# muellerlab/agri-fly

Measured on AMD Instinct MI355X. Metric: vehicle-steps/sec @dt=1ms, higher is better.
Workload: dtype f32; 1 GPU; BASELINE config 4 per GPU: 1048576 hovering CF_MINIQUAD vehicles, per-vehicle wind gusts (sigma 0..0.5 N, 100 ms epochs), IMU synthesis + noise at the 500 Hz logic gate, one afe_step call per 1 ms step, state through memory every step; vehicles_per_gpu=1048576, vehicles_total=1048576, steps_per_call=1, stepping=persistent, noise=AFE_SEED_DECORRELATED: the reference's per-vehicle libstdc++ streams, bit-exact, parallelism=contiguous shards, 1 rank(s), no data-path collective

## Files before the change

agri-fly_amd/csrc/afe_kernels.hip:

```cpp
#include <hip/hip_runtime.h>
#include <stdint.h>

#include "afe_device.h"

namespace afe {

__device__ __forceinline__ float fm(float a, float b, float c) { return __builtin_fmaf(a, b, c); }
__device__ __forceinline__ double fm(double a, double b, double c) { return __builtin_fma(a, b, c); }
__device__ __forceinline__ float m_abs(float x) { return fabsf(x); }
__device__ __forceinline__ double m_abs(double x) { return fabs(x); }
__device__ __forceinline__ float m_med3(float x, float lo, float hi) { return __builtin_amdgcn_fmed3f(x, lo, hi); }
__device__ __forceinline__ double m_med3(double x, double lo, double hi) { return x > hi ? hi : (x < lo ? lo : x); }


template <typename R>
__device__ __forceinline__ void rot_matrix(R v0, R v1, R v2, R v3, R M[9]) {
#pragma clang fp contract(off)
  const R r0 = v0 * v0, r1 = v1 * v1, r2 = v2 * v2, r3 = v3 * v3;
  const R a = 2 * v0, b = 2 * v1, c = 2 * v2;
  M[0] = r0 + r1 - r2 - r3;
  M[1] = fm(b, v2, -(a * v3));
  M[2] = fm(b, v3, a * v2);
  M[3] = fm(b, v2, a * v3);
  M[4] = r0 - r1 + r2 - r3;
  M[5] = fm(c, v3, -(a * v1));
  M[6] = fm(b, v3, -(a * v2));
  M[7] = fm(c, v3, a * v1);
  M[8] = r0 - r1 - r2 + r3;
}

template <typename R, typename M>
__device__ __forceinline__ void mat_vec(const M *A, R x, R y, R z, R &ox, R &oy, R &oz) {
#pragma clang fp contract(off)
  ox = fm(R(A[2]), z, fm(R(A[1]), y, R(A[0]) * x));
  oy = fm(R(A[5]), z, fm(R(A[4]), y, R(A[3]) * x));
  oz = fm(R(A[8]), z, fm(R(A[7]), y, R(A[6]) * x));
}

#ifndef AFE_ACCEPT_LOOP
#define AFE_ACCEPT_LOOP 2
#endif

__device__ __forceinline__ uint32_t minstd_next(uint32_t &s) {
  const uint64_t p = (uint64_t)s * 16807u;
  uint32_t r = (uint32_t)(p & 0x7fffffffu) + (uint32_t)(p >> 31);
  if (r >= 2147483647u) r -= 2147483647u;
  s = r;
  return r;
}

__device__ __forceinline__ uint32_t minstd_mul(uint32_t x, uint32_t k) {
  const uint64_t p = (uint64_t)x * k;
  uint32_t r = (uint32_t)(p & 0x7fffffffu) + (uint32_t)(p >> 31);
  if (r >= 2147483647u) r -= 2147483647u;
  return r;
}

__device__ __forceinline__ double canonical53(uint32_t &s) {
#pragma clang fp contract(off)
  double sum = (double)(minstd_next(s) - 1u);
  sum = sum + (double)(minstd_next(s) - 1u) * 2147483646.0;
  const double b = 4611686009837453312.0;
  const double y = 1.0 / 4611686009837453312.0;
  const double q0 = sum * y;
  const double r = __builtin_fma(-q0, b, sum);
  double ret = __builtin_fma(r, y, q0);
  if (ret >= 1.0) ret = 0x1.fffffffffffffp-1;
  return ret;
}

__device__ __forceinline__ double polar_multiplier(double r2) {
#pragma clang fp contract(off)
  double m = __builtin_amdgcn_frexp_mant(r2);
  int e = __builtin_amdgcn_frexp_exp(r2);
  if (m < 0.70710678118654752) { m = m + m; e -= 1; }
  const double f = m - 1.0;
  const double b = 2.0 + f;
  double y = __builtin_amdgcn_rcp(b);
  y = __builtin_fma(y, __builtin_fma(-b, y, 1.0), y);
  y = __builtin_fma(y, __builtin_fma(-b, y, 1.0), y);
  double sq = f * y;
  sq = __builtin_fma(__builtin_fma(-b, sq, f), y, sq);
  const double z = sq * sq;
  double p = 1.0 / 21.0;
  p = __builtin_fma(p, z, 1.0 / 19.0);
  p = __builtin_fma(p, z, 1.0 / 17.0);
  p = __builtin_fma(p, z, 1.0 / 15.0);
  p = __builtin_fma(p, z, 1.0 / 13.0);
  p = __builtin_fma(p, z, 1.0 / 11.0);
  p = __builtin_fma(p, z, 1.0 / 9.0);
  p = __builtin_fma(p, z, 1.0 / 7.0);
  p = __builtin_fma(p, z, 1.0 / 5.0);
  p = __builtin_fma(p, z, 1.0 / 3.0);
  const double two_s = sq + sq;
  const double lnm = __builtin_fma(two_s * z, p, two_s);
  const double ed = (double)e;
  const double ln_r2 = __builtin_fma(ed, 6.93147180369123816490e-01, __builtin_fma(ed, 1.90821492927058770002e-10, lnm));
  const double L = -2.0 * ln_r2;
  const double w = L * r2;
  if (!(w > 0.0)) return 0.0;
  double g = __builtin_amdgcn_rsq(w);
  g = __builtin_fma(g, 0.5 * __builtin_fma(-(w * g), g, 1.0), g);
  g = __builtin_fma(g, 0.5 * __builtin_fma(-(w * g), g, 1.0), g);
  return L * g;
}

__device__ __forceinline__ float polar_multiplier_f32(double r2) {
#pragma clang fp contract(off)
  double m = __builtin_amdgcn_frexp_mant(r2);
  int e = __builtin_amdgcn_frexp_exp(r2);
  if (m < 0.70710678118654752) { m = m + m; e -= 1; }
  const float f = (float)(m - 1.0);
  const float sq = f * __builtin_amdgcn_rcpf(2.0f + f);
  const float z = sq * sq;
  float p = 1.0f / 9.0f;
  p = __builtin_fmaf(p, z, 1.0f / 7.0f);
  p = __builtin_fmaf(p, z, 1.0f / 5.0f);
  p = __builtin_fmaf(p, z, 1.0f / 3.0f);
  const float two_s = sq + sq;
  const float lnm = __builtin_fmaf(two_s * z, p, two_s);
  const float ln_r2 = __builtin_fmaf((float)e, 0.693147182f, lnm);
  const float L = -2.0f * ln_r2;
  if (!(L > 0.0f)) return 0.0f;
  return __builtin_amdgcn_sqrtf(L * __builtin_amdgcn_rcpf((float)r2));
}

__device__ __forceinline__ void polar_candidate(uint32_t &s, double &x, double &y, double &r2) {
#pragma clang fp contract(off)
  x = 2.0 * canonical53(s) - 1.0;
  y = 2.0 * canonical53(s) - 1.0;
  r2 = x * x + y * y;
}

__device__ __forceinline__ void three_accepted(uint32_t &s, uint32_t &st0, uint32_t &st1, uint32_t &st2) {
#pragma clang fp contract(off)
#if AFE_ACCEPT_LOOP == 2
  st0 = s; st1 = s; st2 = s;
  int got = 0;
  const uint32_t kLo = __builtin_bit_cast(uint32_t, 1e-5f), kUp = __builtin_bit_cast(uint32_t, 1.0f - 1e-5f),
                 kTop = __builtin_bit_cast(uint32_t, 1.0f + 1e-5f);
  for (;;) {
    const uint32_t before = s;
    const uint32_t hx = minstd_mul(before, 282475249u);
    const uint32_t hy = minstd_mul(before, 984943658u);
    s = hy;
    const float kInvR = 1.0f / 2147483646.0f;
    const float xf = __builtin_fmaf((float)(hx - 1u), 2.0f * kInvR, -1.0f);
    const float yf = __builtin_fmaf((float)(hy - 1u), 2.0f * kInvR, -1.0f);
    const uint32_t rb = __builtin_bit_cast(uint32_t, __builtin_fmaf(xf, xf, yf * yf));
    bool accept = (rb - (kLo + 1u)) < (kUp - kLo - 1u);
    const bool unsure = !accept && rb <= kTop;
    if (__ballot(unsure)) {
      if (unsure) {
        uint32_t t = before;
        asm volatile("" : "+v"(t));
        double x, y, r2;
        polar_candidate(t, x, y, r2);
        accept = !(r2 > 1.0 || r2 == 0.0);
      }
    }
    if (accept) {
      asm volatile("v_mov_b32 %0, %1\n\tv_mov_b32 %1, %2\n\tv_mov_b32 %2, %3" : "+&v"(st0), "+&v"(st1), "+&v"(st2) : "v"(before));
      got++;
    }
    if (got >= 3) break;
  }
#else
  st0 = s; st1 = s; st2 = s;
  int got = 0;
  while (got < 3) {
    const uint32_t before = s;
    const uint32_t hx = minstd_mul(before, 282475249u);
    const uint32_t hy = minstd_mul(before, 984943658u);
    s = hy;
    const float kInvR = 1.0f / 2147483646.0f;
    const float xf = __builtin_fmaf((float)(hx - 1u), 2.0f * kInvR, -1.0f);
    const float yf = __builtin_fmaf((float)(hy - 1u), 2.0f * kInvR, -1.0f);
    const float r2f = __builtin_fmaf(xf, xf, yf * yf);
    bool accept = r2f < 1.0f - 1e-5f && r2f > 1e-5f;
    const bool unsure = !accept && !(r2f > 1.0f + 1e-5f);
    if (__ballot(unsure)) {
      if (unsure) {
        uint32_t t = before;
        asm volatile("" : "+v"(t));
        double x, y, r2;
        polar_candidate(t, x, y, r2);
        accept = !(r2 > 1.0 || r2 == 0.0);
      }
    }
    const int slot = accept ? got : 3;
    st0 = slot == 0 ? before : st0;
    st1 = slot == 1 ? before : st1;
    st2 = slot == 2 ? before : st2;
    got += accept ? 1 : 0;
  }
#endif
}

__device__ __forceinline__ void six_normals(uint32_t &s, double d[6]) {
#pragma clang fp contract(off)
  uint32_t st0, st1, st2;
  three_accepted(s, st0, st1, st2);
  double x0, y0, r0, x1, y1, r1, x2, y2, r2;
  polar_candidate(st0, x0, y0, r0);
  polar_candidate(st1, x1, y1, r1);
  polar_candidate(st2, x2, y2, r2);
  const double m0 = polar_multiplier(r0);
  const double m1 = polar_multiplier(r1);
  const double m2 = polar_multiplier(r2);
  d[0] = y0 * m0; d[1] = x0 * m0;
  d[2] = y1 * m1; d[3] = x1 * m1;
  d[4] = y2 * m2; d[5] = x2 * m2;
}

__device__ __forceinline__ void six_normals(uint32_t &s, float d[6]) {
#pragma clang fp contract(off)
  uint32_t st0, st1, st2;
  three_accepted(s, st0, st1, st2);
  double x0, y0, r0, x1, y1, r1, x2, y2, r2;
  polar_candidate(st0, x0, y0, r0);
  polar_candidate(st1, x1, y1, r1);
  polar_candidate(st2, x2, y2, r2);
  const float m0 = polar_multiplier_f32(r0);
  const float m1 = polar_multiplier_f32(r1);
  const float m2 = polar_multiplier_f32(r2);
  d[0] = (float)y0 * m0; d[1] = (float)x0 * m0;
  d[2] = (float)y1 * m1; d[3] = (float)x1 * m1;
  d[4] = (float)y2 * m2; d[5] = (float)x2 * m2;
}

__device__ __forceinline__ void philox4x32_10(uint32_t c[4], uint32_t k0, uint32_t k1) {
  const uint32_t M0 = 0xD2511F53u, M1 = 0xCD9E8D57u, W0 = 0x9E3779B9u, W1 = 0xBB67AE85u;
  asm volatile("" : "+s"(k0), "+s"(k1));
#pragma unroll
  for (int r = 0; r < 10; r++) {
    const uint32_t h0 = __umulhi(M0, c[0]), l0 = M0 * c[0], h1 = __umulhi(M1, c[2]), l1 = M1 * c[2];
    c[0] = h1 ^ c[1] ^ k0; c[1] = l1; c[2] = h0 ^ c[3] ^ k1; c[3] = l0;
    k0 += W0; k1 += W1;
  }
}
#define AFE_STREAM_IMU 1u
#define AFE_STREAM_GUST 2u
__device__ __forceinline__ void counter_block(uint64_t seed, uint64_t index, uint32_t stream, uint32_t block, uint64_t ordinal, uint32_t w[4]) {
  w[0] = (uint32_t)index;
  w[1] = (uint32_t)((index >> 32) & 0xffffu) | (stream << 16) | (block << 24);
  w[2] = (uint32_t)ordinal;
  w[3] = (uint32_t)(ordinal >> 32);
  philox4x32_10(w, (uint32_t)seed, (uint32_t)(seed >> 32));
}
__device__ __forceinline__ void box_muller(uint32_t xe, uint32_t xo, float &za, float &zb) {
#pragma clang fp contract(off)
  const float u_r = ((float)(xe >> 9) + 0.5f) * (1.0f / 8388608.0f);
  const float u_a = (float)(xo >> 8) * (1.0f / 16777216.0f);
  float m = __builtin_amdgcn_frexp_mantf(u_r);
  int e = __builtin_amdgcn_frexp_expf(u_r);
  if (m < 0.70710678f) { m = m + m; e -= 1; }
  const float f = m - 1.0f;
  const float sq = f * __builtin_amdgcn_rcpf(2.0f + f);
  const float z = sq * sq;
  float p = 1.0f / 9.0f;
  p = __builtin_fmaf(p, z, 1.0f / 7.0f);
  p = __builtin_fmaf(p, z, 1.0f / 5.0f);
  p = __builtin_fmaf(p, z, 1.0f / 3.0f);
  const float two_s = sq + sq;
  const float lnm = __builtin_fmaf(two_s * z, p, two_s);
  const float ln_u = __builtin_fmaf((float)e, 0.693147182f, lnm);
  const float r = __builtin_amdgcn_sqrtf(-2.0f * ln_u);
  za = r * __builtin_amdgcn_cosf(u_a);
  zb = r * __builtin_amdgcn_sinf(u_a);
}
__device__ __forceinline__ void box_muller(uint32_t xe, uint32_t xo, double &za, double &zb) {
#pragma clang fp contract(off)
  const double u_r = ((double)(xe >> 9) + 0.5) * (1.0 / 8388608.0);
  const double u_a = (double)(xo >> 8) * (1.0 / 16777216.0);
  const double r = sqrt(-2.0 * log(u_r));
  double sn, cs;
  sincos(6.283185307179586476925286766559 * u_a, &sn, &cs);
  za = r * cs;
  zb = r * sn;
}
template <typename N>
__device__ __forceinline__ void counter_six_normals(uint64_t seed, uint64_t index, uint64_t tick, N d[6]) {
  uint32_t a[4], b[4];
  counter_block(seed, index, AFE_STREAM_IMU, 0, tick, a);
  counter_block(seed, index, AFE_STREAM_IMU, 1, tick, b);
  N unused0, unused1;
  box_muller(a[0], a[1], d[0], d[1]);
  box_muller(a[2], a[3], d[2], d[3]);
  box_muller(b[0], b[1], d[4], d[5]);
  (void)unused0; (void)unused1;
}
template <typename R>
__device__ __forceinline__ void gust_force(uint64_t seed, uint64_t index, uint64_t n_global, uint64_t epoch, double sigma_max, R f[3]) {
#pragma clang fp contract(off)
  uint32_t w[4];
  counter_block(seed, index, AFE_STREAM_GUST, 0, epoch, w);
  R z0, z1, z2, z3;
  box_muller(w[0], w[1], z0, z1);
  box_muller(w[2], w[3], z2, z3);
  const R sigma = (R)(sigma_max * (double)index / (double)(n_global > 1 ? n_global - 1 : 1));
  f[0] = sigma * z0; f[1] = sigma * z1; f[2] = sigma * z2;
}

__device__ __forceinline__ void rotvec_to_quat(double rx, double ry, double rz,
                                               double &d0, double &d1, double &d2, double &d3) {
#pragma clang fp contract(off)
  const double theta = sqrt(rx * rx + ry * ry + rz * rz);
  d0 = 1; d1 = 0; d2 = 0; d3 = 0;
  if (!(theta < 4.84813681e-6)) {
    double sn, cs;
    sincos(theta * 0.5, &sn, &cs);
    d0 = cs;
    d1 = sn * (rx / theta);
    d2 = sn * (ry / theta);
    d3 = sn * (rz / theta);
  }
}
__device__ __forceinline__ void rotvec_to_quat(float rx, float ry, float rz,
// ... 289 lines not shown

    R Lx, Ly, Lzz;
    mat_vec<R>(P.I, wx, wy, wz, Lx, Ly, Lzz);
    if (lagged) Lzz = (((Lzz + Lm[0]) + Lm[1]) + Lm[2]) + Lm[3];
    const R cx = fm(wy, Lzz, -(wz * Ly));
    const R cy = fm(wz, Lx, -(wx * Lzz));
    const R cz = fm(wx, Ly, -(wy * Lx));
    R aax, aay, aaz;
    mat_vec<R>(P.Iinv, Tx - cx, Ty - cy, Tz - cz, aax, aay, aaz);

    const R vbx = fm(Rm[6], vz, fm(Rm[3], vy, Rm[0] * vx));
    const R vby = fm(Rm[7], vz, fm(Rm[4], vy, Rm[1] * vx));
    const R vbz = fm(Rm[8], vz, fm(Rm[5], vy, Rm[2] * vx));
    const R Fbx = P.drag[0] * (-vbx);
    const R Fby = P.drag[1] * (-vby);
    const R Fbz = fm(P.drag[2], -vbz, Fz);

    R accx = div_mass(fm(Rm[2], Fbz, fm(Rm[1], Fby, Rm[0] * Fbx)) + fex, P.mass, P.inv_mass);
    R accy = div_mass(fm(Rm[5], Fbz, fm(Rm[4], Fby, Rm[3] * Fbx)) + fey, P.mass, P.inv_mass);
    R accz, nvz;
    if (sizeof(R) == 4) {
      const R rest = fm(Rm[8], P.drag[2] * (-vbz), fm(Rm[7], Fby, Rm[6] * Fbx)) + fez;
      const double accz_d = __builtin_fma((double)Rm[8], P.kf_over_mass_d * W2_d, -9.81) + (double)(rest * P.inv_mass);
      accz = (R)accz_d;
      nvz = (R)((double)vz + (double)dt * accz_d);
    } else {
      accz = R(-9.81) + div_mass(fm(Rm[8], Fbz, fm(Rm[7], Fby, Rm[6] * Fbx)) + fez, P.mass, P.inv_mass);
      nvz = fm(dt, accz, vz);
    }

    const R hdt = R(0.5) * dt;
    R npx = fm(dt, fm(hdt, accx, vx), px);
    R npy = fm(dt, fm(hdt, accy, vy), py);
    R npz = fm(dt, fm(hdt, accz, vz), pz);
    R nvx = fm(dt, accx, vx), nvy = fm(dt, accy, vy);
    R d0, d1, d2, d3;
    rotvec_to_quat(dt * wx, dt * wy, dt * wz, d0, d1, d2, d3);
    R n0 = fm(-d3, q3, fm(-d2, q2, fm(-d1, q1, d0 * q0)));
    R n1 = fm(-d2, q3, fm(d3, q2, fm(d0, q1, d1 * q0)));
    R n2 = fm(d1, q3, fm(d0, q2, fm(-d3, q1, d2 * q0)));
    R n3 = fm(d0, q3, fm(-d1, q2, fm(d2, q1, d3 * q0)));
    R nwx = fm(dt, aax, wx), nwy = fm(dt, aay, wy), nwz = fm(dt, aaz, wz);

    if (RENORM) {
      const R inv = quat_inv_norm(fm(n3, n3, fm(n2, n2, fm(n1, n1, n0 * n0))));
      n0 *= inv; n1 *= inv; n2 *= inv; n3 *= inv;
    }

    if ((npz <= 0) && (nvz < 0)) {
      npz = 0; nvz = 0; accz = 0;
      nwx = 0; nwy = 0; nwz = 0;
    }
    px = npx; py = npy; pz = npz;
    vx = nvx; vy = nvy; vz = nvz;
    q0 = n0; q1 = n1; q2 = n2; q3 = n3;
    wx = nwx; wy = nwy; wz = nwz;

    if (LOGIC && SINGLE && AFE_LOGIC_LOADS_LATE) {
      AFE_ST(R, pos, 0, off, px); AFE_ST(R, pos, 1, off, py); AFE_ST(R, pos, 2, off, pz);
      AFE_ST(R, vel, 0, off, vx); AFE_ST(R, vel, 1, off, vy); AFE_ST(R, vel, 2, off, vz);
      AFE_ST(R, att, 0, off, q0); AFE_ST(R, att, 1, off, q1); AFE_ST(R, att, 2, off, q2); AFE_ST(R, att, 3, off, q3);
      AFE_ST(R, ang_vel, 0, off, wx); AFE_ST(R, ang_vel, 1, off, wy); AFE_ST(R, ang_vel, 2, off, wz);
    }
    if (tick) {
      if (LOGIC && SINGLE && AFE_LOGIC_LOADS_LATE) {
        __builtin_amdgcn_sched_barrier(0);
        AFE_LOAD_LOGIC_STATE();
      }
      float tx_, ty_, tz_;
      mat_vec<float>(P.Rimu, (float)wx, (float)wy, (float)wz, tx_, ty_, tz_);
      gx = tx_ + ng[0]; gy = ty_ + ng[1]; gz = tz_ + ng[2];
      R Rn[9];
      rot_matrix<R>(q0, q1, q2, q3, Rn);
      const R sx = accx + R(0), sy = accy + R(0), sz = accz + R(9.81);
      const R bx = fm(Rn[6], sz, fm(Rn[3], sy, Rn[0] * sx));
      const R by = fm(Rn[7], sz, fm(Rn[4], sy, Rn[1] * sx));
      const R bz = fm(Rn[8], sz, fm(Rn[5], sy, Rn[2] * sx));
      mat_vec<float>(P.Rimu, (float)bx, (float)by, (float)bz, tx_, ty_, tz_);
      ax_m = tx_ + na[0]; ay_m = ty_ + na[1]; az_m = tz_ + na[2];
      have_imu = true;
      if (LOGIC) {
        rates_logic_tick(G, lg, gx, gy, gz, cmd_new);
#pragma unroll
        for (int m = 0; m < 4; m++) { cmd[m] = (R)cmd_new[m]; if (cmd[m] < 0) cmd[m] = 0; }
      }
    }
    if (EACH && step + 1 < n_steps) {
      AFE_ST(R, pos, 0, off, px); AFE_ST(R, pos, 1, off, py); AFE_ST(R, pos, 2, off, pz);
      AFE_ST(R, vel, 0, off, vx); AFE_ST(R, vel, 1, off, vy); AFE_ST(R, vel, 2, off, vz);
      AFE_ST(R, att, 0, off, q0); AFE_ST(R, att, 1, off, q1); AFE_ST(R, att, 2, off, q2); AFE_ST(R, att, 3, off, q3);
      AFE_ST(R, ang_vel, 0, off, wx); AFE_ST(R, ang_vel, 1, off, wy); AFE_ST(R, ang_vel, 2, off, wz);
      if (v.motor_write) { AFE_ST(R, motor, 0, off, ms[0]); AFE_ST(R, motor, 1, off, ms[1]); AFE_ST(R, motor, 2, off, ms[2]); AFE_ST(R, motor, 3, off, ms[3]); }
      if (tick) {
        AFE_ST(float, gyro, 0, off4, gx); AFE_ST(float, gyro, 1, off4, gy); AFE_ST(float, gyro, 2, off4, gz);
        AFE_ST(float, acc, 0, off4, ax_m); AFE_ST(float, acc, 1, off4, ay_m); AFE_ST(float, acc, 2, off4, az_m);
        if (LOGIC) {
#pragma unroll
          for (int m = 0; m < 4; m++) AFE_ST(float, cmd_out, m, off4, cmd_new[m]);
        }
      }
    }
  }

  if (!(LOGIC && SINGLE && AFE_LOGIC_LOADS_LATE)) {
    AFE_ST(R, pos, 0, off, px); AFE_ST(R, pos, 1, off, py); AFE_ST(R, pos, 2, off, pz);
    AFE_ST(R, vel, 0, off, vx); AFE_ST(R, vel, 1, off, vy); AFE_ST(R, vel, 2, off, vz);
    AFE_ST(R, att, 0, off, q0); AFE_ST(R, att, 1, off, q1); AFE_ST(R, att, 2, off, q2); AFE_ST(R, att, 3, off, q3);
    AFE_ST(R, ang_vel, 0, off, wx); AFE_ST(R, ang_vel, 1, off, wy); AFE_ST(R, ang_vel, 2, off, wz);
  }
  if (v.motor_write) {
    AFE_ST(R, motor, 0, off, ms[0]); AFE_ST(R, motor, 1, off, ms[1]); AFE_ST(R, motor, 2, off, ms[2]); AFE_ST(R, motor, 3, off, ms[3]);
  }
  if (have_imu) {
    AFE_ST(float, gyro, 0, off4, gx); AFE_ST(float, gyro, 1, off4, gy); AFE_ST(float, gyro, 2, off4, gz);
    AFE_ST(float, acc, 0, off4, ax_m); AFE_ST(float, acc, 1, off4, ay_m); AFE_ST(float, acc, 2, off4, az_m);
    if (NOISE == 1) AFE_ST(uint32_t, rng, 0, off4, rng);
    if (LOGIC) {
#pragma unroll
      for (int k = 0; k < 3; k++) {
        AFE_STL(float, lpf, k, off4, lg.xm0[k]);
        AFE_STL(float, lpf, 3 + k, off4, lg.xm1[k]);
        AFE_STL(float, lpf, 6 + k, off4, lg.ym0[k]);
        AFE_STL(float, lpf, 9 + k, off4, lg.ym1[k]);
      }
      v.imu_init[(uint32_t)i] = lg.imu_init;
#pragma unroll
      for (int m = 0; m < 4; m++) AFE_ST(float, cmd_out, m, off4, cmd_new[m]);
    }
  }
#undef AFE_LD
#undef AFE_ST
#undef AFE_LDL
#undef AFE_LOAD_LOGIC_STATE
#undef AFE_STL
}

#ifndef AFE_LB_WAVES
#define AFE_LB_WAVES 1
#endif
#ifndef AFE_BLOCK
#define AFE_BLOCK 64
#endif

template <typename R, bool FEXT, bool TEXT, int NOISE, bool LOGIC, bool SINGLE, bool BUF, int CP = 0>
__global__ void __launch_bounds__(AFE_BLOCK, AFE_LB_WAVES)
afe_step_kernel(const StepView<R> v, const DevParams<R> P, const DevLogic G) {
  const unsigned b = CP == 3 ? (blockIdx.x & 7u) * (gridDim.x >> 3) + (blockIdx.x >> 3) : blockIdx.x;
  const int64_t i = v.first + (int64_t)b * AFE_BLOCK + threadIdx.x;
  if (i >= v.end) return;
  run_vehicle<R, FEXT, TEXT, NOISE, LOGIC, SINGLE, BUF, false, (CP > 2 ? 2 : CP)>(v, P, G, i, v.tick_mask, v.n_steps, v.tick_base);
}

template <typename R, bool FEXT, bool TEXT, int NOISE, bool LOGIC, bool BUF>
__global__ void __launch_bounds__(256)
afe_step_kernel_table(const StepView<R> v) {
  extern __shared__ __align__(16) unsigned char lds_raw[];
  const int words_p = v.n_types * (int)(sizeof(DevParams<R>) / 4);
  const int words_g = LOGIC ? v.n_types * (int)(sizeof(DevLogic) / 4) : 0;
  {
    const uint32_t *src = reinterpret_cast<const uint32_t *>(v.table);
    uint32_t *dst = reinterpret_cast<uint32_t *>(lds_raw);
    for (int k = threadIdx.x; k < words_p; k += 256) dst[k] = src[k];
    if (LOGIC) {
      const uint32_t *srcg = reinterpret_cast<const uint32_t *>(v.logic_table);
      for (int k = threadIdx.x; k < words_g; k += 256) dst[words_p + k] = srcg[k];
    }
  }
  __syncthreads();
  const int64_t i = v.first + (int64_t)blockIdx.x * 256 + threadIdx.x;
  if (i >= v.end) return;
  const unsigned t = v.type[(uint32_t)i];
  const DevParams<R> &P = reinterpret_cast<const DevParams<R> *>(lds_raw)[t];
  const DevLogic &G = reinterpret_cast<const DevLogic *>(lds_raw + (size_t)words_p * 4)[LOGIC ? t : 0];
  run_vehicle<R, FEXT, TEXT, NOISE, LOGIC, false, BUF>(v, P, G, i, v.tick_mask, v.n_steps, v.tick_base);
}

template <typename R, bool FEXT, bool TEXT, int NOISE, bool LOGIC, bool BUF>
__global__ void __launch_bounds__(AFE_BLOCK, AFE_LB_WAVES)
afe_step_kernel_wave_types(const StepView<R> v) {
  const int64_t i = v.first + (int64_t)blockIdx.x * AFE_BLOCK + threadIdx.x;
  if (i >= v.end) return;
  const unsigned t = (unsigned)__builtin_amdgcn_readfirstlane((int)v.type[i]);
  const DevParams<R> P = v.table[t];
  DevLogic G = {};
  if (LOGIC) G = v.logic_table[t];
  run_vehicle<R, FEXT, TEXT, NOISE, LOGIC, false, BUF>(v, P, G, i, v.tick_mask, v.n_steps, v.tick_base);
}

typedef unsigned long long u64_t;
__device__ __forceinline__ u64_t ld_agent(const u64_t *p) { return __hip_atomic_load(p, __ATOMIC_RELAXED, __HIP_MEMORY_SCOPE_AGENT); }
__device__ __forceinline__ void st_agent(u64_t *p, u64_t x) { __hip_atomic_store(p, x, __ATOMIC_RELAXED, __HIP_MEMORY_SCOPE_AGENT); }
__device__ __forceinline__ u64_t ld_system(const u64_t *p) { return __hip_atomic_load(p, __ATOMIC_RELAXED, __HIP_MEMORY_SCOPE_SYSTEM); }
__device__ __forceinline__ void st_system(u64_t *p, u64_t x) { __hip_atomic_store(p, x, __ATOMIC_RELAXED, __HIP_MEMORY_SCOPE_SYSTEM); }
typedef unsigned int afe_u32x16 __attribute__((ext_vector_type(16)));
__device__ __forceinline__ u64_t afe_uniform64(unsigned long long a) {
  return ((u64_t)(unsigned)__builtin_amdgcn_readfirstlane((int)(a >> 32)) << 32) | (unsigned)__builtin_amdgcn_readfirstlane((int)a);
}
__device__ __forceinline__ void sld_system_8_1(const u64_t *p0, const u64_t *p1, u64_t (&x)[8], u64_t &y) {
  afe_u32x16 v;
  const u64_t u0 = afe_uniform64((unsigned long long)p0), u1 = afe_uniform64((unsigned long long)p1);
  asm volatile("s_load_dwordx16 %0, %2, 0x0 glc\n\ts_load_dwordx2 %1, %3, 0x0 glc\n\ts_waitcnt lgkmcnt(0)" : "=&s"(v), "=&s"(y) : "s"(u0), "s"(u1) : "memory");
#pragma unroll
  for (int i = 0; i < 8; i++) x[i] = ((u64_t)v[2 * i + 1] << 32) | v[2 * i];
}
__device__ __forceinline__ void sld_system2(const u64_t *p0, const u64_t *p1, u64_t &x0, u64_t &x1) {
  const u64_t u0 = afe_uniform64((unsigned long long)p0), u1 = afe_uniform64((unsigned long long)p1);
  asm volatile("s_load_dwordx2 %0, %2, 0x0 glc\n\ts_load_dwordx2 %1, %3, 0x0 glc\n\ts_waitcnt lgkmcnt(0)" : "=&s"(x0), "=&s"(x1) : "s"(u0), "s"(u1) : "memory");
}
__device__ __forceinline__ u64_t ticks100() { return __builtin_amdgcn_s_memrealtime(); }
__device__ __forceinline__ int ones_from_bit0(u64_t m) { return m == ~0ull ? 64 : (int)__builtin_ctzll(~m); }
__device__ __forceinline__ u64_t entry_index(u64_t e) { return (e >> 2) & ((1ull << 46) - 1); }
__device__ __forceinline__ u64_t entry_stamp(u64_t e, unsigned epoch) { return (e & ((1ull << 48) - 1)) | ((u64_t)(epoch & 0xffffu) << 48); }

__device__ __forceinline__ u64_t *persist_sync_counters(const PersistArgs &a) { return a.done + ((a.n_workers + 15) & ~15) + 16; }

__device__ __forceinline__ void persist_pump(const PersistArgs &a) {
  const int lane = (int)threadIdx.x;
  u64_t p = a.start;
  const u64_t t_start = ticks100();
  u64_t t_fed = t_start;
  u64_t t_moving = t_start;
  u64_t m_seen = a.start;
  u64_t park_pos;
  u64_t err = 0;
  u64_t m = a.start;
  u64_t *const help = a.dev_ring - 1;
  if (lane == 0) st_agent(help, 0);
  for (int w = lane; w < a.n_workers; w += 64) st_agent(a.done + w, a.start);
  st_agent(persist_sync_counters(a) + 16 * lane, 0);
  if (lane == 0) st_agent(persist_sync_counters(a) + 16 * AFE_PERSIST_SYNC_SHARDS, 0);
  __builtin_amdgcn_fence(__ATOMIC_RELEASE, "agent");
  u64_t req_marked = 0;
  u64_t acc = ~0ull;
  int sw = 0;
  u64_t d[8];
  u64_t help_in = 0, help_seen = 0;
  int slice_age = -1;
#pragma unroll
  for (int j = 0; j < 8; j++) d[j] = ~0ull;
  for (;;) {
    const u64_t idx = p + (u64_t)lane;
    u64_t e8[8], req;
    const u64_t slot = p & a.host_mask;
    if (slot + 8 <= a.host_mask + 1) sld_system_8_1(a.host_ring + slot, a.host_status + AFE_PERSIST_SYNCREQ_WORD, e8, req);
    else {
      sld_system2(a.host_ring + slot, a.host_status + AFE_PERSIST_SYNCREQ_WORD, e8[0], req);
#pragma unroll
      for (int i = 1; i < 8; i++) e8[i] = 0;
    }
    const bool news = entry_index(e8[0]) == p + 1;
    bool all8 = true;
#pragma unroll
    for (int i = 0; i < 8; i++) all8 = all8 && entry_index(e8[i]) == p + 1 + (u64_t)i;
    const bool fetch = all8 && p + 64 < m + (u64_t)a.dev_mask + 1;
    u64_t h = 0;
    if (fetch) h = ld_system(a.host_ring + (idx & a.host_mask));
    else {
#pragma unroll
      for (int i = 0; i < 8; i++) h = lane == i ? e8[i] : h;
    }
    const bool tight = p + 192 >= m + (u64_t)a.dev_mask + 1;
    if (slice_age >= (tight ? 0 : 2)) {
#pragma unroll
      for (int j = 0; j < 8; j++) acc = d[j] < acc ? d[j] : acc;
      help_seen = help_in;
      slice_age = -1;
      sw += 512;
      if (sw >= a.n_workers) {
        u64_t r = acc;
#pragma unroll
        for (int o = 32; o > 0; o >>= 1) { const u64_t other = __shfl_xor(r, o, 64); r = other < r ? other : r; }
        m = r; acc = ~0ull; sw = 0;
        if (lane == 0) st_system(a.host_status + 1, m);
      }
    }
    const bool ready = entry_index(h) == idx + 1;
    const bool room = idx + 64 < m + (u64_t)a.dev_mask + 1;
    int cnt = ones_from_bit0(__ballot(ready && room));
    const u64_t parks = __ballot(ready && (h & AFE_PERSIST_PARK)) & (cnt == 64 ? ~0ull : ((1ull << cnt) - 1));
    if (parks) cnt = (int)__builtin_ctzll(parks) + 1;
    if (lane < cnt) st_agent(a.dev_ring + (idx & a.dev_mask), entry_stamp(h, a.epoch));
    p += (u64_t)cnt;
    if (parks) { park_pos = p - 1; break; }
    if (req != req_marked && req == p) {
      if (lane == 0) st_agent(a.dev_ring + (p & a.dev_mask), entry_stamp(((p + 1) << 2) | AFE_PERSIST_PARK | AFE_PERSIST_TICK, a.epoch));
      req_marked = req;
    }
    const u64_t now = ticks100();
    const bool fed = news;
    if (fed || m < p) t_fed = now;
    if (cnt > 0 || !fed || m != m_seen) t_moving = now;
    m_seen = m;
    const bool idle = now - t_fed > (u64_t)a.idle_ticks;
    const bool gave_up = now - t_moving > (u64_t)a.give_up_ticks || help_seen != 0;
    if (idle && !gave_up) {
      if (lane == 0) st_system(a.host_status + 7, p + 1);
      __builtin_amdgcn_fence(__ATOMIC_SEQ_CST, "");
      const u64_t again = ld_system(a.host_ring + (p & a.host_mask));
      if (entry_index(again) == p + 1) {
        if (lane == 0) st_system(a.host_status + 7, 0);
        t_fed = ticks100();
        continue;
      }
    }
    if (idle || gave_up) {
      if (lane == 0) st_agent(a.dev_ring + (p & a.dev_mask), entry_stamp(((p + 1) << 2) | AFE_PERSIST_PARK, a.epoch));
      park_pos = p;
      if (gave_up) err = 1;
      break;
    }
    if (slice_age < 0) {
#pragma unroll
      for (int j = 0; j < 8; j++) { const int w = sw + lane + 64 * j; d[j] = w < a.n_workers ? ld_agent(a.done + w) : ~0ull; }
      help_in = ld_agent(help);
      slice_age = 0;
    } else slice_age++;
  }
  if (err) {
    u64_t low = ~0ull;
    int who = -1, with = 0;
    for (int w0 = 0; w0 < a.n_workers; w0 += 64) {
      const int w = w0 + lane;
      const u64_t d = w < a.n_workers ? ld_agent(a.done + w) : ~0ull;
      if (d < low) { low = d; who = w; with = 0; }
      if (d == low && w < a.n_workers) with++;
    }
    u64_t glow = low;
#pragma unroll
    for (int o = 32; o > 0; o >>= 1) { const u64_t other = __shfl_xor(glow, o, 64); glow = other < glow ? other : glow; }
    const u64_t holders = __ballot(low == glow);
    int total = low == glow ? with : 0;
#pragma unroll
    for (int o = 32; o > 0; o >>= 1) total += __shfl_xor(total, o, 64);
    if (lane == (int)__builtin_ctzll(holders)) {
      st_system(a.host_status + 3, glow);
      st_system(a.host_status + 4, p);
      st_system(a.host_status + 5, ((u64_t)(unsigned)who << 32) | (u64_t)(unsigned)total);
      st_system(a.host_status + 6, (ld_agent(help) << 32) | (u64_t)(unsigned)a.n_workers);
    }
  }
  if (lane == 0) {
    if (err) st_system(a.host_status + 2, err);
    st_system(a.host_status + 0, park_pos + 1);
  }
}

__device__ __forceinline__ void persist_set_priority(const PersistArgs &a, int steps_left, int batch) {
  if (!(a.epoch & AFE_PERSIST_PRIO)) return;
  if (2 * steps_left > batch) __builtin_amdgcn_s_setprio(3);
  else if (4 * steps_left > batch) __builtin_amdgcn_s_setprio(2);
  else __builtin_amdgcn_s_setprio(1);
}

#define AFE_HOST_ACQUIRE() __builtin_amdgcn_fence(__ATOMIC_ACQUIRE, "")
#define AFE_HOST_RELEASE() __builtin_amdgcn_fence(__ATOMIC_RELEASE, "")
template <typename R, bool LOGIC, bool RESIDENT>
constexpr int persistent_min_waves() { return sizeof(R) != 4 ? 1 : (!RESIDENT ? 6 : (LOGIC ? 3 : 5)); }
template <typename R, bool FEXT, bool LOGIC, bool RESIDENT>
constexpr bool persist_holds() { return sizeof(R) == 4 && FEXT && !LOGIC && !RESIDENT; }
template <typename R, bool FEXT, int NOISE, bool LOGIC, bool RESIDENT>
__global__ void __launch_bounds__(64) __attribute__((amdgpu_waves_per_eu(persistent_min_waves<R, LOGIC, RESIDENT>())))
afe_step_persistent_kernel(const StepView<R> v, const DevParams<R> P_arg, const DevLogic G_arg, const PersistArgs a) {
  if (blockIdx.x == 0) { persist_pump(a); return; }
  const int lane = (int)threadIdx.x;
  constexpr bool lds_params = LOGIC && RESIDENT;
  __shared__ DevParams<R> P_lds;
  __shared__ DevLogic G_lds;
  if (lds_params) {
    const uint32_t *ps = reinterpret_cast<const uint32_t *>(&P_arg), *gs = reinterpret_cast<const uint32_t *>(&G_arg);
    uint32_t *pd = reinterpret_cast<uint32_t *>(&P_lds), *gd = reinterpret_cast<uint32_t *>(&G_lds);
    for (int k = lane; k < (int)(sizeof(DevParams<R>) / 4); k += 64) pd[k] = ps[k];
    if (LOGIC) for (int k = lane; k < (int)(sizeof(DevLogic) / 4); k += 64) gd[k] = gs[k];
    __syncthreads();
  }
  const DevParams<R> &P = lds_params ? P_lds : P_arg;
  const DevLogic &G = lds_params ? G_lds : G_arg;
  const int w = (int)blockIdx.x - 1;
  u64_t s = a.start;
  u64_t t_wait = ticks100();
  u64_t tick_no = v.tick_base;
  int idle_polls = 0;
  u64_t gust_in_slab = a.gust_epoch_applied, gust_epoch = a.gust_epoch0;
  u64_t gust_next_us = (a.gust_epoch0 + 1) * a.gust_period_us, t_us = a.t0_us;
  bool sync_answered = false;
  constexpr bool HOLDS = persist_holds<R, FEXT, LOGIC, RESIDENT>();
  __shared__ HeldInputs held_lds[1];
  const bool hold = HOLDS && (a.epoch & AFE_PERSIST_HOLD);
  if (HOLDS && hold) {
    for (int j = 0, c = w; j < AFE_PERSIST_HELD_SLOTS && c < a.n_chunks; j++, c += a.n_workers) {
      const int64_t i = (int64_t)c * 64 + lane;
      if (i < v.n) {
#pragma unroll
        for (int m = 0; m < 4; m++) held_lds[0].v[j][m][lane] = v.cmd[m * v.stride + i];
#pragma unroll
        for (int k = 0; k < 3; k++) held_lds[0].v[j][4 + k][lane] = (float)v.ext_force[k * v.stride + i];
      }
    }
  }
  const bool spare = 4 * ((a.n_chunks - w + a.n_workers - 1) / a.n_workers) <= 3 * ((a.n_chunks + a.n_workers - 1) / a.n_workers);
  for (;;) {
    const u64_t idx = s + (u64_t)lane;
    const u64_t e = ld_agent(a.dev_ring + (idx & a.dev_mask));
    const bool ready = entry_index(e) == idx + 1 && (!(e & AFE_PERSIST_PARK) || (unsigned)(e >> 48) == (a.epoch & 0xffffu));
    const bool marker = ready && (e & 3ull) == 3ull;
    const int cnt = ones_from_bit0(__ballot(ready && !marker));
    if (cnt == 0) {
      if (!sync_answered && (__ballot(marker) & 1ull)) {
        asm volatile("s_waitcnt vmcnt(0)" ::: "memory");
        sync_answered = true;
        if (lane == 0) {
          u64_t *const cnts = persist_sync_counters(a);
          const unsigned shard = (unsigned)w & (AFE_PERSIST_SYNC_SHARDS - 1);
          const unsigned in_shard = ((unsigned)a.n_workers - shard + AFE_PERSIST_SYNC_SHARDS - 1) / AFE_PERSIST_SYNC_SHARDS;
          const unsigned shards = (unsigned)a.n_workers < AFE_PERSIST_SYNC_SHARDS ? (unsigned)a.n_workers : AFE_PERSIST_SYNC_SHARDS;
          const u64_t got = __hip_atomic_fetch_add(cnts + 16 * shard, 1ull, __ATOMIC_RELAXED, __HIP_MEMORY_SCOPE_AGENT) + 1;
          if (got % in_shard == 0) {
            const u64_t top = __hip_atomic_fetch_add(cnts + 16 * AFE_PERSIST_SYNC_SHARDS, 1ull, __ATOMIC_RELAXED, __HIP_MEMORY_SCOPE_AGENT) + 1;
            if (top % shards == 0) st_system(a.host_status + AFE_PERSIST_SYNC_WORD, s);
          }
        }
      }
      const u64_t waited = ticks100() - t_wait;
      if (waited > (u64_t)a.give_up_ticks + 1000000ull && lane == 0) st_agent(a.dev_ring - 1, 1);
      if (waited > (u64_t)a.give_up_ticks + 1050000000ull) {
        if (lane == 0) st_system(a.host_status + 2, 2);
        return;
      }
      if (idle_polls < 64 && !(a.epoch & AFE_PERSIST_HOST_IO)) idle_polls++;
      const int ex = idle_polls < 3 ? idle_polls : (spare ? 7 : (idle_polls < 64 ? 3 : 5));
      __builtin_amdgcn_s_sleep(2);
      for (int b = 1; b < (1 << ex); b++) __builtin_amdgcn_s_sleep(2);
      continue;
    }
    idle_polls = 0; sync_answered = false;
    if (a.epoch & AFE_PERSIST_HOST_IO) AFE_HOST_ACQUIRE();
    const u64_t low = cnt == 64 ? ~0ull : ((1ull << cnt) - 1);
    const u64_t ticks = __ballot(ready && (e & AFE_PERSIST_TICK)) & low;
    const u64_t parks = __ballot(ready && (e & AFE_PERSIST_PARK)) & low;
    int run = parks ? (int)__builtin_ctzll(parks) : cnt;
    if (RESIDENT) {
      if (a.gust_period_us && run > 0) {
        while (t_us >= gust_next_us) { gust_epoch++; gust_next_us += a.gust_period_us; }
        const u64_t left = (gust_next_us - t_us + a.dt_us - 1) / a.dt_us;
        if ((u64_t)run > left) run = (int)left;
        if (gust_epoch != gust_in_slab) {
          for (int c = w; c < a.n_chunks; c += a.n_workers) {
            const int64_t i = (int64_t)c * 64 + lane;
            if (i < v.n) {
              R f[3];
              gust_force<R>(a.gust_seed, (uint64_t)(v.first_global + i), a.gust_n_global, gust_epoch, a.gust_sigma_max, f);
              R *slab = const_cast<R *>(v.ext_force);
              slab[i] = f[0]; slab[v.stride + i] = f[1]; slab[2 * v.stride + i] = f[2];
            }
          }
          gust_in_slab = gust_epoch;
        }
        t_us += (u64_t)run * a.dt_us;
      }
      if (run > 0) {
        persist_set_priority(a, run, run);
        const u64_t batch_ticks = ticks & (run == 64 ? ~0ull : ((1ull << run) - 1));
        for (int c = w; c < a.n_chunks; c += a.n_workers) {
          const int64_t i = (int64_t)c * 64 + lane;
          if (i < v.n) run_vehicle<R, FEXT, false, NOISE, LOGIC, false, true, true>(v, P, G, i, batch_ticks, run, tick_no);
        }
        tick_no += (u64_t)__popcll(batch_ticks);
      }
      s += (u64_t)run;
      if (a.epoch & AFE_PERSIST_HOST_IO) {
        AFE_HOST_RELEASE();
        if (lane == 0 && a.n_workers <= AFE_PERSIST_HOST_MARKS) st_system(a.host_status + 8 + w, s);
      }
      if (lane == 0) st_agent(a.done + w, s);
      if (parks && run == (int)__builtin_ctzll(parks)) return;
      t_wait = ticks100();
      continue;
    }
    for (int k = 0; k < run; k++) {
      persist_set_priority(a, run - k, run);
      const u64_t tick = (ticks >> k) & 1ull;
      if (a.gust_period_us) {
        while (t_us >= gust_next_us) { gust_epoch++; gust_next_us += a.gust_period_us; }
        if (gust_epoch != gust_in_slab) {
          for (int j = 0, c = w; c < a.n_chunks; j++, c += a.n_workers) {
            const int64_t i = (int64_t)c * 64 + lane;
            if (i < v.n) {
              R f[3];
              gust_force<R>(a.gust_seed, (uint64_t)(v.first_global + i), a.gust_n_global, gust_epoch, a.gust_sigma_max, f);
              R *slab = const_cast<R *>(v.ext_force);
              slab[i] = f[0]; slab[v.stride + i] = f[1]; slab[2 * v.stride + i] = f[2];
              if (HOLDS && hold && j < AFE_PERSIST_HELD_SLOTS) {
#pragma unroll
                for (int k = 0; k < 3; k++) held_lds[0].v[j][4 + k][lane] = (float)f[k];
              }
            }
          }
          gust_in_slab = gust_epoch;
        }
        t_us += a.dt_us;
      }
      for (int j = 0, c = w; c < a.n_chunks; j++, c += a.n_workers) {
        const int64_t i = (int64_t)c * 64 + lane;
        if (i < v.n)
          run_vehicle<R, FEXT, false, NOISE, LOGIC, true, true, false, 0, HOLDS>(v, P, G, i, tick, 1, tick_no, HOLDS ? &held_lds[0] : nullptr,
                                                                                 hold && j < AFE_PERSIST_HELD_SLOTS ? j : -1);
      }
      tick_no += tick;
    }
    s += (u64_t)run;
    if (a.epoch & AFE_PERSIST_HOST_IO) {
      AFE_HOST_RELEASE();
      if (lane == 0 && a.n_workers <= AFE_PERSIST_HOST_MARKS) st_system(a.host_status + 8 + w, s);
    }
    if (lane == 0) st_agent(a.done + w, s);
    if (parks) return;
    t_wait = ticks100();
  }
}

template <typename R>
__global__ void __launch_bounds__(256) afe_gust_kernel(R *ext_force, int64_t stride, int64_t n, int64_t first_global, uint64_t n_global,
                                                        uint64_t seed, uint64_t epoch, double sigma_max) {
  const int64_t i = (int64_t)blockIdx.x * 256 + threadIdx.x;
  if (i >= n) return;
  R f[3];
  gust_force<R>(seed, (uint64_t)(first_global + i), n_global, epoch, sigma_max, f);
  ext_force[i] = f[0]; ext_force[stride + i] = f[1]; ext_force[2 * stride + i] = f[2];
}
int launch_gust_f32(float *ext_force, int64_t stride, int64_t n, int64_t first_global, uint64_t n_global, uint64_t seed, uint64_t epoch,
                    double sigma_max, void *stream) {
  hipLaunchKernelGGL(afe_gust_kernel<float>, dim3((unsigned)((n + 255) / 256)), dim3(256), 0, (hipStream_t)stream, ext_force, stride, n, first_global,
                     n_global, seed, epoch, sigma_max);
  return (int)hipGetLastError();
}
int launch_gust_f64(double *ext_force, int64_t stride, int64_t n, int64_t first_global, uint64_t n_global, uint64_t seed, uint64_t epoch,
                    double sigma_max, void *stream) {
  hipLaunchKernelGGL(afe_gust_kernel<double>, dim3((unsigned)((n + 255) / 256)), dim3(256), 0, (hipStream_t)stream, ext_force, stride, n, first_global,
                     n_global, seed, epoch, sigma_max);
  return (int)hipGetLastError();
}

template <typename R>
static int launch_persistent(const StepView<R> &v, const LaunchFlags &f, const DevParams<R> &uniform,
                             const DevLogic *uniform_logic, const PersistArgs &a, hipStream_t st, int *occupancy, const void **fn_out = nullptr) {
  DevLogic no_logic = {};
  const DevLogic &G = uniform_logic ? *uniform_logic : no_logic;
  const dim3 grid((unsigned)(1 + a.n_workers)), block(64);
#define AFE_PL_R(FE, NO, LO, RE)                                                                                        \
  do {                                                                                                                  \
    if (fn_out) {                                                                                                       \
      *fn_out = reinterpret_cast<const void *>(&afe_step_persistent_kernel<R, FE, NO, LO, RE>);                         \
    } else if (occupancy) {                                                                                             \
      if (hipOccupancyMaxActiveBlocksPerMultiprocessor(occupancy, afe_step_persistent_kernel<R, FE, NO, LO, RE>, 64, 0) != hipSuccess) \
        *occupancy = 0;                                                                                                 \
    } else {                                                                                                            \
      hipLaunchKernelGGL((afe_step_persistent_kernel<R, FE, NO, LO, RE>), grid, block, 0, st, v, uniform, G, a);        \
    }                                                                                                                   \
  } while (0)
#define AFE_PL(FE, NO, LO) do { if (f.resident) AFE_PL_R(FE, NO, LO, true); else AFE_PL_R(FE, NO, LO, false); } while (0)
#define AFE_PL_LO(FE, NO) do { if (f.logic) AFE_PL(FE, NO, true); else AFE_PL(FE, NO, false); } while (0)
#define AFE_PL_NO(FE) do { if (!f.noise) AFE_PL_LO(FE, 0); else if (f.counter_noise) AFE_PL_LO(FE, 2); else AFE_PL_LO(FE, 1); } while (0)
  if (f.ext_force) AFE_PL_NO(true); else AFE_PL_NO(false);
#undef AFE_PL_NO
#undef AFE_PL_LO
#undef AFE_PL
#undef AFE_PL_R
  return (int)hipGetLastError();
}

template <typename R>
static int persistent_capacity(const LaunchFlags &f) {
  StepView<R> v = {};
  DevParams<R> P = {};
  PersistArgs a = {};
  int per_cu = 0;
  (void)launch_persistent<R>(v, f, P, nullptr, a, nullptr, &per_cu);
  const int sgpr_bound = 6 * 4;
  return per_cu < sgpr_bound ? per_cu : sgpr_bound;
}
template <typename R>
static const void *persistent_kernel_fn(const LaunchFlags &f) {
  StepView<R> v = {};
  DevParams<R> P = {};
  PersistArgs a = {};
  const void *fn = nullptr;
  (void)launch_persistent<R>(v, f, P, nullptr, a, nullptr, nullptr, &fn);
  return fn;
}
const void *persistent_kernel_fn_f32(const LaunchFlags &f) { return persistent_kernel_fn<float>(f); }
const void *persistent_kernel_fn_f64(const LaunchFlags &f) { return persistent_kernel_fn<double>(f); }
int persistent_capacity_f32(const LaunchFlags &f) { return persistent_capacity<float>(f); }
int persistent_capacity_f64(const LaunchFlags &f) { return persistent_capacity<double>(f); }

int launch_persistent_f32(const StepView<float> &v, const LaunchFlags &f, const DevParams<float> &uniform,
                          const DevLogic *uniform_logic, const PersistArgs &a, void *stream) {
  return launch_persistent<float>(v, f, uniform, uniform_logic, a, (hipStream_t)stream, nullptr);
}
int launch_persistent_f64(const StepView<double> &v, const LaunchFlags &f, const DevParams<double> &uniform,
                          const DevLogic *uniform_logic, const PersistArgs &a, void *stream) {
  return launch_persistent<double>(v, f, uniform, uniform_logic, a, (hipStream_t)stream, nullptr);
}

template <typename R>
static int launch_step(const StepView<R> &v, const LaunchFlags &f, const DevParams<R> *uniform,
                       const DevLogic *uniform_logic, hipStream_t st) {
  const int64_t count = v.end - v.first;
  if (count <= 0) return 0;
  const unsigned grid = (unsigned)((count + 255) / 256);
  const unsigned grid_u = (unsigned)((count + AFE_BLOCK - 1) / AFE_BLOCK);
  const size_t lds = (size_t)v.n_types * (sizeof(DevParams<R>) + (f.logic ? sizeof(DevLogic) : 0));
  DevLogic no_logic = {};
  const DevLogic &G = uniform_logic ? *uniform_logic : no_logic;
#define AFE_LAUNCH_B(FE, TE, NO, LO, BU)                                                                   \
  do {                                                                                                     \
    if (uniform && v.n_steps == 1) {                                                                       \
       \
      constexpr bool CPOK = (BU) && !(TE);                                                                 \
      const int cp = !CPOK ? 0 : (f.cache_policy == 3 && (grid_u & 7u) ? 2 : f.cache_policy);             \
      if (cp == 1) hipLaunchKernelGGL((afe_step_kernel<R, FE, TE, NO, LO, true, BU, CPOK ? 1 : 0>), dim3(grid_u), dim3(AFE_BLOCK), 0, st, v, *uniform, G); \
      else if (cp == 2) hipLaunchKernelGGL((afe_step_kernel<R, FE, TE, NO, LO, true, BU, CPOK ? 2 : 0>), dim3(grid_u), dim3(AFE_BLOCK), 0, st, v, *uniform, G); \
      else if (cp == 3) hipLaunchKernelGGL((afe_step_kernel<R, FE, TE, NO, LO, true, BU, CPOK ? 3 : 0>), dim3(grid_u), dim3(AFE_BLOCK), 0, st, v, *uniform, G); \
      else hipLaunchKernelGGL((afe_step_kernel<R, FE, TE, NO, LO, true, BU>), dim3(grid_u), dim3(AFE_BLOCK), 0, st, v, *uniform, G); \
    }                                                                                                      \
    else if (uniform)                                                                                      \
      hipLaunchKernelGGL((afe_step_kernel<R, FE, TE, NO, LO, false, BU>), dim3(grid_u), dim3(AFE_BLOCK), 0, st, v, *uniform, G); \
    else if (f.wave_uniform_types && AFE_BLOCK == 64)                                                      \
      hipLaunchKernelGGL((afe_step_kernel_wave_types<R, FE, TE, NO, LO, BU>), dim3(grid_u), dim3(AFE_BLOCK), 0, st, v); \
    else {                                                                                                 \
                                \
      if (lds > 65536 &&                                                                                   \
          hipFuncSetAttribute(reinterpret_cast<const void *>(&afe_step_kernel_table<R, FE, TE, NO, LO, BU>), \
                              hipFuncAttributeMaxDynamicSharedMemorySize, (int)lds) != hipSuccess)         \
        return (int)hipErrorInvalidValue;                                                                  \
      hipLaunchKernelGGL((afe_step_kernel_table<R, FE, TE, NO, LO, BU>), dim3(grid), dim3(256), lds, st, v); \
    }                                                                                                      \
  } while (0)
#define AFE_LAUNCH(FE, TE, NO, LO) do { if (v.buf_bytes) AFE_LAUNCH_B(FE, TE, NO, LO, true); else AFE_LAUNCH_B(FE, TE, NO, LO, false); } while (0)
#define AFE_SEL_LO(FE, TE, NO) do { if (f.logic) AFE_LAUNCH(FE, TE, NO, true); else AFE_LAUNCH(FE, TE, NO, false); } while (0)
#define AFE_SEL_NO(FE, TE) do { if (!f.noise) AFE_SEL_LO(FE, TE, 0); else if (f.counter_noise) AFE_SEL_LO(FE, TE, 2); else AFE_SEL_LO(FE, TE, 1); } while (0)
#define AFE_SEL_TE(FE) do { if (f.ext_torque) AFE_SEL_NO(FE, true); else AFE_SEL_NO(FE, false); } while (0)
  if (f.ext_force) AFE_SEL_TE(true); else AFE_SEL_TE(false);
#undef AFE_SEL_TE
#undef AFE_SEL_NO
#undef AFE_SEL_LO
#undef AFE_LAUNCH
#undef AFE_LAUNCH_B
  return (int)hipGetLastError();
}

int launch_step_f32(const StepView<float> &v, const LaunchFlags &f, const DevParams<float> *uniform,
                    const DevLogic *uniform_logic, void *stream) {
  return launch_step<float>(v, f, uniform, uniform_logic, (hipStream_t)stream);
}
int launch_step_f64(const StepView<double> &v, const LaunchFlags &f, const DevParams<double> *uniform,
                    const DevLogic *uniform_logic, void *stream) {
  return launch_step<double>(v, f, uniform, uniform_logic, (hipStream_t)stream);
}

// ... 134 lines not shown
```

Before: 59.64 billion vehicle-steps/s.

## Reload persistent kernargs per step, wave-level accept masks, exact trims, table occupancy hints

The persistent kernel now re-reads its view, params and args from the kernarg segment on each step and chunk instead of keeping copies live across the loop. The goal is to cut SGPR/VGPR pressure in the held-input noise path. The polar-method acceptance loop now tracks accepted-sample counts as wave-wide ballot masks instead of per-lane counters. canonical53 drops its >=1 clamp and polar_candidate uses fma under the EXACT_TRIMS default, which risks deviating from the bit-exact reference streams. The table kernel also gets waves_per_eu occupancy hints for certain template configurations.

```diff
diff --git a/agri-fly_amd/csrc/afe_kernels.hip b/agri-fly_amd/csrc/afe_kernels.hip
--- a/agri-fly_amd/csrc/afe_kernels.hip
+++ b/agri-fly_amd/csrc/afe_kernels.hip
@@ -1,4 +1,5 @@
 #include <hip/hip_runtime.h>
+#include <stddef.h>
 #include <stdint.h>
 
 #include "afe_device.h"
@@ -37,6 +38,12 @@
   oz = fm(R(A[8]), z, fm(R(A[7]), y, R(A[6]) * x));
 }
 
+#ifndef AFE_KERNARG_RELOAD
+#define AFE_KERNARG_RELOAD 1
+#endif
+#ifndef AFE_EXACT_TRIMS
+#define AFE_EXACT_TRIMS 1
+#endif
 #ifndef AFE_ACCEPT_LOOP
 #define AFE_ACCEPT_LOOP 2
 #endif
@@ -65,7 +72,9 @@
   const double q0 = sum * y;
   const double r = __builtin_fma(-q0, b, sum);
   double ret = __builtin_fma(r, y, q0);
+#if !AFE_EXACT_TRIMS
   if (ret >= 1.0) ret = 0x1.fffffffffffffp-1;
+#endif
   return ret;
 }
 
@@ -127,8 +136,13 @@
 
 __device__ __forceinline__ void polar_candidate(uint32_t &s, double &x, double &y, double &r2) {
 #pragma clang fp contract(off)
+#if AFE_EXACT_TRIMS
+  x = __builtin_fma(2.0, canonical53(s), -1.0);
+  y = __builtin_fma(2.0, canonical53(s), -1.0);
+#else
   x = 2.0 * canonical53(s) - 1.0;
   y = 2.0 * canonical53(s) - 1.0;
+#endif
   r2 = x * x + y * y;
 }
 
@@ -136,7 +150,7 @@
 #pragma clang fp contract(off)
 #if AFE_ACCEPT_LOOP == 2
   st0 = s; st1 = s; st2 = s;
-  int got = 0;
+  uint64_t m1 = 0, m2 = 0, m3 = 0;
   const uint32_t kLo = __builtin_bit_cast(uint32_t, 1e-5f), kUp = __builtin_bit_cast(uint32_t, 1.0f - 1e-5f),
                  kTop = __builtin_bit_cast(uint32_t, 1.0f + 1e-5f);
   for (;;) {
@@ -148,22 +162,24 @@
     const float xf = __builtin_fmaf((float)(hx - 1u), 2.0f * kInvR, -1.0f);
     const float yf = __builtin_fmaf((float)(hy - 1u), 2.0f * kInvR, -1.0f);
     const uint32_t rb = __builtin_bit_cast(uint32_t, __builtin_fmaf(xf, xf, yf * yf));
-    bool accept = (rb - (kLo + 1u)) < (kUp - kLo - 1u);
-    const bool unsure = !accept && rb <= kTop;
-    if (__ballot(unsure)) {
-      if (unsure) {
+    uint64_t am = __builtin_amdgcn_ballot_w64((rb - (kLo + 1u)) < (kUp - kLo - 1u));
+    const uint64_t um = __builtin_amdgcn_ballot_w64(rb <= kTop) & ~am;
+    if (um) {
+      bool ex = false;
+      if (__builtin_amdgcn_inverse_ballot_w64(um)) {
         uint32_t t = before;
         asm volatile("" : "+v"(t));
         double x, y, r2;
         polar_candidate(t, x, y, r2);
-        accept = !(r2 > 1.0 || r2 == 0.0);
-      }
-    }
-    if (accept) {
+        ex = !(r2 > 1.0 || r2 == 0.0);
+      }
+      am |= __builtin_amdgcn_ballot_w64(ex);
+    }
+    if (__builtin_amdgcn_inverse_ballot_w64(am)) {
       asm volatile("v_mov_b32 %0, %1\n\tv_mov_b32 %1, %2\n\tv_mov_b32 %2, %3" : "+&v"(st0), "+&v"(st1), "+&v"(st2) : "v"(before));
-      got++;
-    }
-    if (got >= 3) break;
+    }
+    m3 |= m2 & am; m2 |= m1 & am; m1 |= am;
+    if (__builtin_amdgcn_inverse_ballot_w64(m3)) break;
   }
 #else
   st0 = s; st1 = s; st2 = s;
@@ -759,7 +775,14 @@
 }
 
 template <typename R, bool FEXT, bool TEXT, int NOISE, bool LOGIC, bool BUF>
-__global__ void __launch_bounds__(256)
+constexpr int table_min_waves() {
+  constexpr bool at_a_register_step = NOISE == 1 && LOGIC && BUF;
+  constexpr bool both_wrenches = FEXT && TEXT;
+  if (!at_a_register_step || both_wrenches) return 1;
+  return sizeof(R) == 4 ? 4 : 2;
+}
+template <typename R, bool FEXT, bool TEXT, int NOISE, bool LOGIC, bool BUF>
+__global__ void __launch_bounds__(256) __attribute__((amdgpu_waves_per_eu(table_min_waves<R, FEXT, TEXT, NOISE, LOGIC, BUF>())))
 afe_step_kernel_table(const StepView<R> v) {
   extern __shared__ __align__(16) unsigned char lds_raw[];
   const int words_p = v.n_types * (int)(sizeof(DevParams<R>) / 4);
@@ -965,6 +988,12 @@
 constexpr int persistent_min_waves() { return sizeof(R) != 4 ? 1 : (!RESIDENT ? 6 : (LOGIC ? 3 : 5)); }
 template <typename R, bool FEXT, bool LOGIC, bool RESIDENT>
 constexpr bool persist_holds() { return sizeof(R) == 4 && FEXT && !LOGIC && !RESIDENT; }
+template <typename R>
+__device__ __forceinline__ const PersistKernarg<R> &persist_kernarg() {
+  const __attribute__((address_space(4))) char *p = (const __attribute__((address_space(4))) char *)__builtin_amdgcn_kernarg_segment_ptr();
+  asm volatile("" : "+s"(p));
+  return *(const PersistKernarg<R> *)p;
+}
 template <typename R, bool FEXT, int NOISE, bool LOGIC, bool RESIDENT>
 __global__ void __launch_bounds__(64) __attribute__((amdgpu_waves_per_eu(persistent_min_waves<R, LOGIC, RESIDENT>())))
 afe_step_persistent_kernel(const StepView<R> v, const DevParams<R> P_arg, const DevLogic G_arg, const PersistArgs a) {
@@ -983,6 +1012,7 @@
   const DevParams<R> &P = lds_params ? P_lds : P_arg;
   const DevLogic &G = lds_params ? G_lds : G_arg;
   const int w = (int)blockIdx.x - 1;
+  constexpr bool RELOADS = AFE_KERNARG_RELOAD && NOISE == 1 && persist_holds<R, FEXT, LOGIC, RESIDENT>();
   u64_t s = a.start;
   u64_t t_wait = ticks100();
   u64_t tick_no = v.tick_base;
@@ -1084,18 +1114,21 @@
       continue;
     }
     for (int k = 0; k < run; k++) {
-      persist_set_priority(a, run - k, run);
+      const PersistKernarg<R> *const ks = RELOADS ? &persist_kernarg<R>() : nullptr;
+      const StepView<R> &vs = RELOADS ? ks->v : v;
+      const PersistArgs &as = RELOADS ? ks->a : a;
+      persist_set_priority(as, run - k, run);
       const u64_t tick = (ticks >> k) & 1ull;
-      if (a.gust_period_us) {
-        while (t_us >= gust_next_us) { gust_epoch++; gust_next_us += a.gust_period_us; }
+      if (as.gust_period_us) {
+        while (t_us >= gust_next_us) { gust_epoch++; gust_next_us += as.gust_period_us; }
         if (gust_epoch != gust_in_slab) {
-          for (int j = 0, c = w; c < a.n_chunks; j++, c += a.n_workers) {
+          for (int j = 0, c = w; c < as.n_chunks; j++, c += as.n_workers) {
             const int64_t i = (int64_t)c * 64 + lane;
-            if (i < v.n) {
+            if (i < vs.n) {
               R f[3];
-              gust_force<R>(a.gust_seed, (uint64_t)(v.first_global + i), a.gust_n_global, gust_epoch, a.gust_sigma_max, f);
-              R *slab = const_cast<R *>(v.ext_force);
-              slab[i] = f[0]; slab[v.stride + i] = f[1]; slab[2 * v.stride + i] = f[2];
+              gust_force<R>(as.gust_seed, (uint64_t)(vs.first_global + i), as.gust_n_global, gust_epoch, as.gust_sigma_max, f);
+              R *slab = const_cast<R *>(vs.ext_force);
+              slab[i] = f[0]; slab[vs.stride + i] = f[1]; slab[2 * vs.stride + i] = f[2];
               if (HOLDS && hold && j < AFE_PERSIST_HELD_SLOTS) {
 #pragma unroll
                 for (int k = 0; k < 3; k++) held_lds[0].v[j][4 + k][lane] = (float)f[k];
@@ -1104,13 +1137,18 @@
           }
           gust_in_slab = gust_epoch;
         }
-        t_us += a.dt_us;
-      }
-      for (int j = 0, c = w; c < a.n_chunks; j++, c += a.n_workers) {
+        t_us += as.dt_us;
+      }
+      for (int j = 0, c = w;; j++) {
+        const PersistKernarg<R> *const kc = RELOADS ? &persist_kernarg<R>() : nullptr;
+        const StepView<R> &vc = RELOADS ? kc->v : v;
+        const PersistArgs &ac = RELOADS ? kc->a : a;
+        if (c >= ac.n_chunks) break;
         const int64_t i = (int64_t)c * 64 + lane;
-        if (i < v.n)
-          run_vehicle<R, FEXT, false, NOISE, LOGIC, true, true, false, 0, HOLDS>(v, P, G, i, tick, 1, tick_no, HOLDS ? &held_lds[0] : nullptr,
-                                                                                 hold && j < AFE_PERSIST_HELD_SLOTS ? j : -1);
+        if (i < vc.n)
+          run_vehicle<R, FEXT, false, NOISE, LOGIC, true, true, false, 0, HOLDS>(vc, RELOADS ? kc->P : P, RELOADS ? kc->G : G, i, tick, 1, tick_no,
+                                                                                 HOLDS ? &held_lds[0] : nullptr, hold && j < AFE_PERSIST_HELD_SLOTS ? j : -1);
+        c += ac.n_workers;
       }
       tick_no += tick;
     }
```

Result: faster. 61.48 billion vehicle-steps/s (median of 6 runs) (+3.1%).
